# JunzheJosephZhu/DenseMatcher

Hardware: AMD Instinct MI355X
Metric: mesh-pairs/sec at N=2048 D=768 k=128 (higher is better)
Workload: dtype f16; 1 GPU; configs[1]: batch=64 pairs, N=2048, D=768, k=128 functional-map solve; pairs_per_gpu=64, N=2048, D=768, k=128, basis_dtype=float64, parallelism=pairs sharded over 1 GPU(s), one process per GPU, no data-path collective, process_group_size=1

## Files before the change

densematcher_amd/csrc/dm_ctx.hip:

```cpp
#include <stdarg.h>

#include "dm_internal.h"

int dm_fail(dm_ctx* ctx, int code, const char* fmt, ...) {
    char buf[1024];
    va_list ap;
    va_start(ap, fmt);
    vsnprintf(buf, sizeof(buf), fmt, ap);
    va_end(ap);
    if (ctx) ctx->err = buf;
    return code;
}

static thread_local std::string g_create_err = "null context";

static int create_fail(const char* what, hipError_t e) {
    char buf[512];
    snprintf(buf, sizeof(buf), "dm_create: %s%s%s", what, e != hipSuccess ? ": " : "", e != hipSuccess ? hipGetErrorString(e) : "");
    g_create_err = buf;
    return DM_EHIP;
}

extern "C" int dm_create(int device, void* hip_stream, dm_ctx** out) {
    if (!out) return DM_EINVAL;
// ... 11 lines not shown
        char buf[300];
        snprintf(buf, sizeof(buf), "device is %s, libdensematch is built for gfx950 only", prop.gcnArchName);
        return create_fail(buf, hipSuccess);
    }
    dm_ctx* ctx = new dm_ctx();
    ctx->n_cu = prop.multiProcessorCount;
    ctx->device = device;
    ctx->stream = (hipStream_t)hip_stream;
    *out = ctx;
    return DM_OK;
}

extern "C" int dm_destroy(dm_ctx* ctx) {
    if (!ctx) return DM_EINVAL;
    (void)hipSetDevice(ctx->device);
    (void)hipStreamSynchronize(ctx->stream);
    for (hipEvent_t e : ctx->prof_events) (void)hipEventDestroy(e);
    if (ctx->ws) (void)hipFree(ctx->ws);
    if (ctx->gram_keep) (void)hipFree(ctx->gram_keep);
    for (auto& e : ctx->stats) { if (e.buf[0]) (void)hipFree(e.buf[0]); }
    if (ctx->pinned_words) (void)hipHostFree(ctx->pinned_words);
    if (ctx->pinned_event) (void)hipEventDestroy(ctx->pinned_event);
    delete ctx;
    return DM_OK;
}

int dm_pinned_words(dm_ctx* ctx, int32_t** words, hipEvent_t* ev) {
    if (!ctx->pinned_words) DM_CHECK_HIP(ctx, hipHostMalloc((void**)&ctx->pinned_words, 64 * sizeof(int32_t), hipHostMallocDefault));
    if (!ctx->pinned_event) DM_CHECK_HIP(ctx, hipEventCreateWithFlags(&ctx->pinned_event, hipEventDisableTiming));
    *words = ctx->pinned_words; *ev = ctx->pinned_event;
    return DM_OK;
}

#ifdef DM_EXPERIMENTS
#include <stdlib.h>
int dm_knob(const char* env_name, int dflt) {
    const char* e = getenv(env_name);
    return e ? atoi(e) : dflt;
}
#endif

extern "C" int dm_set_option(dm_ctx* ctx, const char* name, int value) {
    if (!ctx || !name) return DM_EINVAL;
    const std::string n = name;
    if (n == "simnn_pipe") ctx->opt_simnn_pipe = value;
    else if (n == "knn_split") ctx->opt_knn_split = value;
    else if (n == "solve_packed") ctx->opt_solve_packed = value;
    else if (n == "solve_reg") ctx->opt_solve_reg = value;
    else if (n == "simnn_band") ctx->opt_simnn_band = value;
    else if (n == "simnn_big") ctx->opt_simnn_big = value;
    else if (n == "simnn_prio") ctx->opt_simnn_prio = value;
    else if (n == "fit_mfma") ctx->opt_fit_mfma = value;
    else if (n == "solve_pcg") ctx->opt_solve_pcg = value;
    else if (n == "basis_stats") { ctx->opt_basis_stats = value; for (auto& e : ctx->stats) e.valid = false; }
    else if (n == "lsa_reg") ctx->opt_lsa_reg = value;
    else if (n == "p2p_split") ctx->opt_p2p_split = value;
    else if (n == "simnn_persist") ctx->opt_simnn_persist = value;
    else if (n == "p2pfm_direct") ctx->opt_p2pfm_direct = value;
    else if (n == "zoomout_fused") ctx->opt_zoomout_fused = value;
    else if (n == "simnn1_wt") ctx->opt_simnn1_wt = value;
    else if (n == "zoomout_sub_fused") ctx->opt_zoomout_sub_fused = value;
    else if (n == "fps_heat_route") ctx->opt_fps_heat_route = value;
    else if (n == "graph_geod_device") ctx->opt_graph_geod_device = value;
    else if (n == "fmn_eig_route") ctx->opt_fmn_eig_route = value;
    else if (n == "proj_onepass") ctx->opt_proj_onepass = value;
    else if (n == "energy_keep_gram") { ctx->opt_energy_keep_gram = value; ctx->gram_valid = false; }
    else return dm_fail(ctx, DM_EINVAL, "dm_set_option: unknown option '%s'", name);
    return DM_OK;
}

extern "C" const char* dm_last_error(const dm_ctx* ctx) { return ctx ? ctx->err.c_str() : g_create_err.c_str(); }
extern "C" const char* dm_version(void) { return DM_VERSION_STRING; }
extern "C" size_t dm_workspace_bytes(const dm_ctx* ctx) { return ctx ? ctx->ws_bytes : 0; }

dm_ctx::basis_stat* dm_stat_entry(dm_ctx* ctx, const void* ptr, int B, int N, int k, int ld, int esz, int n) {
    for (auto& e : ctx->stats)
        if (e.ptr == ptr && e.B == B && e.N == N && e.k == k && e.ld == ld && e.esz == esz && e.n == n && e.buf[0]) return &e;
    dm_ctx::basis_stat& e = ctx->stats[ctx->stats_next];
    ctx->stats_next = (ctx->stats_next + 1) % 4;
    const size_t need = (size_t)B * n * 8;
    if (!e.buf[0] || (size_t)e.B * e.n * 8 < need) {
        if (e.buf[0]) { (void)hipStreamSynchronize(ctx->stream); (void)hipFree(e.buf[0]); e.buf[0] = e.buf[1] = nullptr; }
        void* p = nullptr;
        if (hipMalloc(&p, 2 * dm_align_up(need)) != hipSuccess) { e.ptr = nullptr; return nullptr; }
        e.buf[0] = (double*)p;
        e.buf[1] = (double*)((char*)p + dm_align_up(need));
    } else {
        e.buf[1] = (double*)((char*)e.buf[0] + dm_align_up(need));
    }
    e.ptr = ptr; e.B = B; e.N = N; e.k = k; e.ld = ld; e.esz = esz; e.n = n; e.cur = 0; e.valid = false;
    return &e;
}

int dm_ws_reserve(dm_ctx* ctx, size_t total_bytes) {
    ctx->ws_off = 0;
    ctx->last_flag_counts = nullptr;
    ctx->last_flag_sets = 0;
    total_bytes = dm_align_up(total_bytes + 4096, 1 << 20);
    if (total_bytes <= ctx->ws_bytes) return DM_OK;
    DM_CHECK_HIP(ctx, hipSetDevice(ctx->device));
    if (ctx->ws) {
        DM_CHECK_HIP(ctx, hipStreamSynchronize(ctx->stream));
        DM_CHECK_HIP(ctx, hipFree(ctx->ws));
        ctx->ws = nullptr;
        ctx->ws_bytes = 0;
    }
// ... 106 lines not shown
```

densematcher_amd/csrc/dm_fmap.hip:

```cpp
#include <stdlib.h>

#include "dm_gemm_f64.h"
#include "dm_internal.h"
#include "dm_pcg.h"

struct OutProj {
    float* direct;
    double* partial;
    int B, k, D;
    __device__ __forceinline__ void store(int b, int split, int m, int c, double v) const {
        if (direct) direct[((long long)b * k + m) * D + c] = (float)v;
        else partial[(((long long)split * B + b) * k + m) * D + c] = v;
    }
};

__global__ __launch_bounds__(256) void splitk_reduce_f32_kernel(const double* __restrict__ partial, int nsplit,
                                                                long long n, float* __restrict__ out) {
    const long long i = (long long)blockIdx.x * 256 + threadIdx.x;
    if (i >= n) return;
    double s = 0.0;
    for (int q = 0; q < nsplit; ++q) s += partial[(long long)q * n + i];
    out[i] = (float)s;
}

// ... 587 lines not shown
                    const double* Tik = T + sl(I, K);
#pragma unroll
                    for (int ii = 0; ii < 16; ++ii) a0 = fma(Tik[k * 16 + ii], xv[I * 16 + ii], a0);
                }
                rhs[K * 16 + k] -= a0;
            }
            __syncthreads();
            for (int q = t; q < r1n * 128; q += 256) reinterpret_cast<f64x2*>(T)[q] = reinterpret_cast<const f64x2*>(my_spill)[q];
            __syncthreads();
            blocked_back_subst(T, TriSlots{}, rhs, xv, NA, t);
            if (t == 0) Crow[0] = ci0;
            for (int c = t; c < n; c += 256) Crow[c + 1] = xv[c];
        } else {
            if (t == 0) atomicMax(&info[b], i + 1);
            for (int c = t; c < k1; c += 256) Crow[c] = (c == 0) ? ci0 : 0.0;
        }
        __syncthreads();
    }
}

#include "dm_chol_reg.h"
#ifndef DM_SOLVE_REG_EV
#define DM_SOLVE_REG_EV 3
#endif

constexpr int solve_reg_ev(int NBT) { return NBT == 8 ? DM_SOLVE_REG_EV : 0; }
constexpr size_t solve_reg_lds(int NBT) {
    const size_t img = (size_t)(NBT * (NBT + 1) / 2) * 256 * sizeof(double);
    const size_t ev = (size_t)4 * dmreg::ev_slot(NBT, solve_reg_ev(NBT), solve_reg_ev(NBT) + 1) * 256 * sizeof(double);
    return img > ev ? img : ev;
}

template <int NBT>
__global__ __launch_bounds__(256, 1) void fmap_solve_reg_kernel(const double* __restrict__ PQ, const double* __restrict__ Timg,
                                                                const double* __restrict__ lam1, const double* __restrict__ lam2,
                                                                const double* __restrict__ c00, double w_lap, int k1, int k2, int NBimg,
                                                                long long nsys, double* __restrict__ C, int32_t* __restrict__ info,
                                                                const int32_t* __restrict__ only_if, int only_ng) {
    const int lane = threadIdx.x & 63, wave = threadIdx.x >> 6;
    const long long sys0 = (long long)blockIdx.x * 4;
    if (only_if && !pcg_flagged(only_if, only_ng, (int)(sys0 / k2)) && !pcg_flagged(only_if, only_ng, (int)(min(sys0 + 3, nsys - 1) / k2))) return;
    const long long sys = min(sys0 + wave, nsys - 1);
    const int b = (int)(sys / k2), i = (int)(sys - (long long)b * k2);
    const int n = k1 - 1, c = lane & 15, g = lane >> 4;
    const double* P = PQ + (long long)b * (k1 + k2) * k1;
    const double* Q = P + (long long)k1 * k1;
    const double* l1 = lam1 + (long long)b * k1;
    const double* l2 = lam2 + (long long)b * k2;
    extern __shared__ __attribute__((aligned(16))) double sh_dyn[];
    f64x4 T[NBT * (NBT + 1) / 2];
    {
        const int nblk = NBimg * (NBimg + 1) / 2;
        const bool one_pair = (int)(sys0 / k2) == (int)(min(sys0 + 3, nsys - 1) / k2);
        const double* imgb = Timg + (long long)b * nblk * 256;
        if (one_pair) {
            const f64x2* src = reinterpret_cast<const f64x2*>(imgb);
            f64x2* dst = reinterpret_cast<f64x2*>(sh_dyn);
            for (int q = threadIdx.x; q < nblk * 128; q += 256) dst[q] = src[q];
            __syncthreads();
        }
#pragma unroll
        for (int I = 0; I < NBT; ++I)
#pragma unroll
            for (int K = 0; K <= I; ++K) {
                f64x4 v = {0.0, 0.0, 0.0, 0.0};
                if (I < NBimg) {
                    if (one_pair) {
#pragma unroll
                        for (int r = 0; r < 4; ++r) v[r] = sh_dyn[dmreg::blk(I, K) * 256 + 64 * r + lane];
                    } else {
#pragma unroll
                        for (int r = 0; r < 4; ++r) v[r] = imgb[(long long)dmreg::blk(I, K) * 256 + 64 * r + lane];
                    }
                }
                T[dmreg::blk(I, K)] = v;
            }
        __syncthreads();
    }
    double mx = -DM_INF_F64;
    for (int q = lane; q < k1; q += 64) mx = fmax(mx, l1[q]);
    for (int q = lane; q < k2; q += 64) mx = fmax(mx, l2[q]);
#pragma unroll
    for (int off = 32; off > 0; off >>= 1) mx = fmax(mx, __shfl_xor(mx, off));
    const double scale = mx;
    const double ci0 = (i == 0) ? c00[b] : 0.0;
    const double l2i = l2[i] / scale;
#pragma unroll
    for (int I = 0; I < NBT; ++I) {
        const int idx = I * 16 + c;
        double pen = 1.0;
        if (idx < n) {
            const double d = l1[idx + 1] / scale - l2i;
            pen = w_lap * (d * d);
        }
        const bool mine = g == (c & 3);
#pragma unroll
        for (int r = 0; r < 4; ++r) {
            const bool hit = mine && (c >> 2) == r;
            const double cur = T[dmreg::blk(I, I)][r];
            T[dmreg::blk(I, I)][r] = hit ? (idx < n ? cur + pen : 1.0) : cur;
        }
    }
    double* Crow = C + ((long long)b * k2 + i) * k1;
    __shared__ double sh_rhs[4][NBT * 16];
    for (int q = lane; q < NBT * 16; q += 64)
        sh_rhs[wave][q] = (q < n) ? Q[(long long)i * k1 + (q + 1)] - (i == 0 ? P[(long long)(q + 1) * k1] * ci0 : 0.0) : 0.0;
    auto rhs = [&](int J) {
        f64x4 rv = {0.0, 0.0, 0.0, 0.0};
        if (c == 0) {
#pragma unroll
            for (int r = 0; r < 4; ++r) rv[r] = sh_rhs[wave][J * 16 + g + 4 * r];
        }
        return rv;
    };
    auto store = [&](int J, const f64x4& x) {
        if (c == 0) {
#pragma unroll
            for (int r = 0; r < 4; ++r) {
                const int ix = J * 16 + g + 4 * r;
                if (ix < n) Crow[ix + 1] = x[r];
            }
        }
    };
    constexpr int EV = solve_reg_ev(NBT);
    if (sys0 + wave >= nsys) return;
    const bool solved = dmreg::solve<NBT, EV>(T, rhs, store, lane, sh_dyn + wave * (dmreg::ev_slot(NBT, EV, EV + 1) * 256));
    if (!solved) {
        if (lane == 0) atomicMax(&info[b], i + 1);
        for (int q = lane; q < k1; q += 64) Crow[q] = (q == 0) ? ci0 : 0.0;
        return;
    }
    if (lane == 0) Crow[0] = ci0;
}

static size_t fmap_solve_ws(const dm_ctx* ctx, int B, int k1, int k2) {
    const size_t pq_bytes = (size_t)B * (k1 + k2) * k1 * 8;
    const int n = k1 - 1, NB = (n + 15) / 16;
    const bool two_phase = (NB == 12 || NB == 13) && !ctx->opt_solve_packed;
    const bool blocked = ((n >= 1 && NB <= 11) && !ctx->opt_solve_packed) || two_phase;
    const size_t img_bytes = blocked ? (size_t)B * (NB * (NB + 1) / 2) * 256 * 8 : 0;
    const int NA = (NB + 1) / 2, grid2 = ctx->n_cu > 0 ? ctx->n_cu : 256;
    const size_t spill_bytes = two_phase ? (size_t)grid2 * (NA * (NA + 1) / 2) * 256 * 8 : 0;
    const size_t pcgs_bytes = (ctx->opt_solve_pcg && n > 128 && n <= 256) ? pcgs_image_bytes(B, n) : 0;
    return dm_align_up(pq_bytes) + dm_align_up(img_bytes) + dm_align_up(spill_bytes) + dm_align_up((size_t)B * dm_cdiv(k2, 32) * 4) + dm_align_up(pcgs_bytes) + 4096;
}

static inline bool fmap_solve_pcg_ok(const dm_ctx* ctx, int k1, int k2) {
    const int n = k1 - 1;
    return ctx->opt_solve_pcg && ctx->opt_solve_reg && !ctx->opt_solve_packed && n >= 65 && n <= 128 && k2 % 4 == 0;
}

template <class OPA, class OPB>
static int fmap_solve_core(dm_ctx* ctx, int B, int k1, int k2, int D, const OPA& opa, const OPB& opb,
                           const double* lam1, const double* lam2, const double* c00, double w_descr, double w_lap,
                           double* C, int32_t* info) {
    const size_t pq_bytes = (size_t)B * (k1 + k2) * k1 * 8;
    const int n = k1 - 1;
    const int NB = (n + 15) / 16;
    const bool two_phase = (NB == 12 || NB == 13) && !ctx->opt_solve_packed;
    const bool blocked = ((n >= 1 && NB <= 11) && !ctx->opt_solve_packed) || two_phase;
    const size_t img_bytes = blocked ? (size_t)B * (NB * (NB + 1) / 2) * 256 * 8 : 0;
    const int NA = (NB + 1) / 2;
    const int grid2 = ctx->n_cu > 0 ? ctx->n_cu : 256;
    const size_t spill_bytes = two_phase ? (size_t)grid2 * (NA * (NA + 1) / 2) * 256 * 8 : 0;
    int rc = DM_OK;
    double* PQ = (double*)dm_ws_take(ctx, pq_bytes);
    double* Timg = blocked ? (double*)dm_ws_take(ctx, img_bytes) : nullptr;
    double* spill = two_phase ? (double*)dm_ws_take(ctx, spill_bytes) : nullptr;
    if (!PQ || (blocked && !Timg) || (two_phase && !spill)) return dm_fail(ctx, DM_ENOMEM, "fmap_solve: workspace not reserved");
    if (blocked) DM_CHECK_HIP(ctx, hipMemsetAsync(Timg, 0, img_bytes, ctx->stream));
    const bool pcg_small = blocked && !two_phase && NB <= 8 && ctx->opt_solve_reg && fmap_solve_pcg_ok(ctx, k1, k2);
    const bool pcg_big = (two_phase || (blocked && NB >= 9)) && ctx->opt_solve_pcg && !ctx->opt_solve_packed;
    if (!pcg_small && !pcg_big) DM_CHECK_HIP(ctx, hipMemsetAsync(info, 0, (size_t)B * sizeof(int32_t), ctx->stream));

    OutScaled out{PQ, (long long)(k1 + k2) * k1, k1, w_descr, Timg, (long long)(NB * (NB + 1) / 2) * 256, k1};
    dim3 grid(dm_cdiv(k1 + k2, NT_T) * dm_cdiv(k1, NT_T), 1, B);
    switch (dm_knob("DM_GRAM_NPRE", 2)) {
        case 1: DM_LAUNCH(ctx, "gram_nt_f64", (gemm_nt_f64<OPA, OPB, OutScaled, 1>), grid, dim3(256), 0, opa, opb, out, k1 + k2, k1, D); break;
        case 4: DM_LAUNCH(ctx, "gram_nt_f64", (gemm_nt_f64<OPA, OPB, OutScaled, 4>), grid, dim3(256), 0, opa, opb, out, k1 + k2, k1, D); break;
        case 3: DM_LAUNCH(ctx, "gram_nt_f64", (gemm_nt_f64<OPA, OPB, OutScaled, 3>), grid, dim3(256), 0, opa, opb, out, k1 + k2, k1, D); break;
        default: DM_LAUNCH(ctx, "gram_nt_f64", (gemm_nt_f64<OPA, OPB, OutScaled, 2, true>), dim3(grid.x * (unsigned)B), dim3(256), 0, opa, opb, out, k1 + k2, k1, D); break;
    }

    const int32_t* only_if_big = nullptr;
    const int only_ng = dm_cdiv(k2, PCG_NS);
    if (pcg_big) {
        int32_t* fb = (int32_t*)dm_ws_take(ctx, (size_t)B * only_ng * 4);
        double* img = (double*)dm_ws_take(ctx, pcgs_image_bytes(B, n));
        if (!fb || !img) return dm_fail(ctx, DM_ENOMEM, "fmap_solve: workspace not reserved");
        const int NTp = (n + 15) / 16, KSP = pcgs_ksp(n), ngroups = dm_cdiv(k2, PCG_NS);
        DM_LAUNCH(ctx, "fmap_solve_pcg_pack", pcgs_pack_kernel, dim3(64, B), dim3(256), 0, (const double*)PQ, k1, k2, NTp, KSP, img);
        const size_t lds_pcg = pcg_lds_bytes(PCGS_NT, PCGS_NW);
        rc = dm_grant_lds(ctx, (const void*)fmap_solve_pcgs_kernel, lds_pcg);
        if (rc) return rc;
        DM_LAUNCH(ctx, "fmap_solve_pcg", fmap_solve_pcgs_kernel, dim3((unsigned)(B * ngroups)), dim3(64 * PCGS_NW), lds_pcg, (const double*)PQ,
                  (const double*)img, lam1, lam2, c00, w_lap, k1, k2, ngroups, NTp, KSP, 1e-22, 48, 6, 3e-4, C, fb, info);
        only_if_big = fb;
    }
    if (two_phase) {
        const int NBr = NB - NA;
        const size_t lds = ((size_t)(NA * (NA + 1) / 2 + NBr * NA + 2) * 256 + 2 * NB * 16 + 8) * sizeof(double) + (96 + 16 + 128) * sizeof(int);
        rc = dm_grant_lds(ctx, (const void*)fmap_solve_2phase_kernel, lds);
        if (rc) return rc;
        const long long nsys = (long long)B * k2;
        DM_LAUNCH(ctx, "fmap_solve_chol", fmap_solve_2phase_kernel, dim3((unsigned)(nsys < grid2 ? nsys : grid2)), dim3(256), lds, PQ, Timg,
                  lam1, lam2, c00, w_lap, k1, k2, NB, B, spill, C, info, only_if_big, only_ng);
        return DM_OK;
    }
    if (blocked && !two_phase && NB <= 8 && ctx->opt_solve_reg) {
        const long long nsys = (long long)B * k2;
        const dim3 grid((unsigned)((nsys + 3) / 4));
        const int32_t* only_if = nullptr;
        if (pcg_small) {
            int32_t* fb = (int32_t*)dm_ws_take(ctx, (size_t)B * only_ng * 4);
            if (!fb) return dm_fail(ctx, DM_ENOMEM, "fmap_solve: workspace not reserved");
            const int ngroups = dm_cdiv(k2, PCG_NS);
            const size_t lds_pcg = pcg_lds_bytes(8, 4);
            rc = dm_grant_lds(ctx, (const void*)fmap_solve_pcg_kernel<8, 4>, lds_pcg);
            if (rc) return rc;
            DM_LAUNCH(ctx, "fmap_solve_pcg", (fmap_solve_pcg_kernel<8, 4>), dim3((unsigned)(B * ngroups)), dim3(256), lds_pcg, PQ, lam1, lam2, c00,
                      w_lap, k1, k2, ngroups, 1e-22, 48, 6, 3e-4, C, fb, info);
            only_if = fb;
        }
#define DM_SOLVE_REG(NBT_)                                                                                             \
        {                                                                                                              \
            rc = dm_grant_lds(ctx, (const void*)fmap_solve_reg_kernel<NBT_>, solve_reg_lds(NBT_));                     \
            if (rc) return rc;                                                                                         \
            DM_LAUNCH(ctx, "fmap_solve_chol", fmap_solve_reg_kernel<NBT_>, grid, dim3(256), solve_reg_lds(NBT_), PQ, Timg, lam1, lam2, \
                      c00, w_lap, k1, k2, NB, nsys, C, info, only_if, only_ng);                                        \
        }
        if (NB <= 2) DM_SOLVE_REG(2)
        else if (NB <= 4) DM_SOLVE_REG(4)
        else if (NB <= 6) DM_SOLVE_REG(6)
        else DM_SOLVE_REG(8)
#undef DM_SOLVE_REG
        return DM_OK;
    }
    if (blocked) {
        const size_t lds = ((size_t)(NB * (NB + 1) / 2 + 2) * 256 + 2 * NB * 16 + 16 + 8) * sizeof(double);
        rc = dm_grant_lds(ctx, (const void*)fmap_solve_blocked_kernel, lds);
        if (rc) return rc;
        DM_LAUNCH(ctx, "fmap_solve_chol", fmap_solve_blocked_kernel, dim3(k2, B), dim3(256), lds, PQ, Timg, lam1, lam2, c00,
                  w_lap, k1, k2, NB, C, info, only_if_big, only_ng);
        return DM_OK;
    }
    const size_t lds = ((size_t)(n + 1) * (n + 2) / 2 + (n + 1 < 16 ? 16 : n + 1) + 4) * sizeof(double);
    rc = dm_grant_lds(ctx, (const void*)fmap_solve_kernel, lds);
    if (rc) return rc;
    DM_LAUNCH(ctx, "fmap_solve_chol", fmap_solve_kernel, dim3(k2, B), dim3(SP_NT), lds, PQ, lam1, lam2, c00, w_lap, k1, k2,
              C, info, dm_knob("DM_SOLVE_DEBUG", 0));
    return DM_OK;
}

extern "C" int dm_fmap_solve(dm_ctx* ctx, int B, int k1, int k2, int D, const float* A, const float* Bm,
                             const double* lam1, const double* lam2, const double* c00, double w_descr, double w_lap,
                             double* C, int32_t* info) {
    if (!ctx) return DM_EINVAL;
    DM_REQUIRE(ctx, B > 0 && k1 > 0 && k2 > 0 && D > 0, "sizes must be positive");
    DM_REQUIRE(ctx, A && Bm && lam1 && lam2 && c00 && C && info, "null pointer");
    DM_REQUIRE(ctx, k1 <= 200, "k1 > 200 does not fit the in-LDS solver");
    DM_REQUIRE(ctx, w_descr >= 0.0 && w_lap >= 0.0 && (w_descr > 0.0 || w_lap > 0.0), "weights must be >= 0 and not both 0");
    DM_CHECK_HIP(ctx, hipSetDevice(ctx->device));
    int rc = dm_ws_reserve(ctx, fmap_solve_ws(ctx, B, k1, k2));
    if (rc) return rc;
    KRowsStackedF32 opa{A, Bm, k1, k2, D};
    KRowsF32 opb{A, (long long)k1 * D, D, k1, D};
    return fmap_solve_core(ctx, B, k1, k2, D, opa, opb, lam1, lam2, c00, w_descr, w_lap, C, info);
}

template <typename TR>
static int fmap_fit_impl(dm_ctx* ctx, int B, int N1, int N2, int D, int k1, int k2, const TR* Phi1, int ld1, const TR* Phi2, int ld2,
                         const TR* mass1, const TR* mass2, const void* F1, const void* F2, const double* lam1, const double* lam2,
                         double w_descr, double w_lap, double* C, int32_t* info) {
    if (!ctx) return DM_EINVAL;
// ... 44 lines not shown
```

densematcher_amd/csrc/dm_internal.h:

```cpp
#pragma once

#include <hip/hip_runtime.h>
#include <stdint.h>
#include <stdio.h>
#include <string.h>

#include <string>
#include <unordered_map>
#include <vector>

#include "densematch.h"

#define DM_VERSION_STRING "densematch 0.5.0 (gfx950, abi 6)"

struct dm_ctx {
    int device = 0;
    hipStream_t stream = nullptr;
    std::string err;

    char* ws = nullptr;
    size_t ws_bytes = 0;
    size_t ws_off = 0;

    std::string prof_name;
    std::vector<hipEvent_t> prof_events;
    std::vector<const char*> prof_names;
    std::vector<const char*> prof_syms;
    size_t prof_used = 0;

    std::unordered_map<const void*, size_t> lds_granted;

    int opt_simnn_pipe = 1;
    int opt_knn_split = 1;
    int opt_solve_packed = 0;
    int opt_proj_onepass = 1;
    int opt_fit_mfma = 1;
    int opt_simnn_prio = 0;
    int opt_simnn_big = 0;
    int opt_simnn_band = 4;
    int opt_lsa_reg = 2;
    int opt_solve_pcg = 1;
    int opt_solve_reg = 1;
    int opt_p2p_split = 2;
    int opt_simnn_persist = 1;
    int opt_p2pfm_direct = 1;
    int opt_simnn1_wt = 4;
    int opt_zoomout_fused = 1;
    int opt_zoomout_sub_fused = 1;
    int opt_fps_heat_route = 0;
    int opt_graph_geod_device = 1;
    int opt_fmn_eig_route = 0;
    int opt_energy_keep_gram = 0;
    double* gram_keep = nullptr;
    size_t gram_keep_bytes = 0;
    const void* gram_key_ptr[5] = {nullptr, nullptr, nullptr, nullptr, nullptr};
    int gram_key_dim[6] = {0, 0, 0, 0, 0, 0};
    bool gram_valid = false;
    bool gram_sums_valid = false;
    int n_cu = 0;
    int32_t* pinned_words = nullptr;
    hipEvent_t pinned_event = nullptr;
    struct basis_stat { const void* ptr = nullptr; int B = 0, N = 0, k = 0, ld = 0, esz = 0, n = 0; double* buf[2] = {nullptr, nullptr}; int cur = 0; bool valid = false; };
    basis_stat stats[4];
    int stats_next = 0;
    int opt_basis_stats = 1;
    const int32_t* last_flag_counts = nullptr;
    int last_flag_sets = 0;
};

#ifdef DM_EXPERIMENTS
int dm_knob(const char* env_name, int dflt);
#else
static inline int dm_knob(const char*, int dflt) { return dflt; }
#endif

int dm_fail(dm_ctx* ctx, int code, const char* fmt, ...);
int dm_pinned_words(dm_ctx* ctx, int32_t** words, hipEvent_t* ev);
int dm_grant_lds(dm_ctx* ctx, const void* func, size_t bytes);

#define DM_CHECK_HIP(ctx, expr)                                                        \
    do {                                                                               \
        hipError_t _e = (expr);                                                        \
        if (_e != hipSuccess)                                                          \
            return dm_fail(ctx, DM_EHIP, "%s failed: %s (%s:%d)", #expr,               \
                           hipGetErrorString(_e), __FILE__, __LINE__);                 \
    } while (0)

#define DM_REQUIRE(ctx, cond, msg)                                                     \
    do {                                                                               \
        if (!(cond)) return dm_fail(ctx, DM_EINVAL, "%s: requirement failed: %s (%s)", \
                                    __func__, #cond, msg);                             \
    } while (0)

int dm_ws_reserve(dm_ctx* ctx, size_t total_bytes);
// ... 187 lines not shown
```

densematcher_amd/csrc/dm_p2p.hip:

```cpp
#include <stdlib.h>

#include "dm_gemm_f64.h"
#include "dm_internal.h"
#include "dm_split.h"
#include "dm_indicator_dev.h"

static inline int pad_to(int x, int m) { return (x + m - 1) / m * m; }

template <typename Tin>
__global__ __launch_bounds__(256) void phiT_kernel(const Tin* __restrict__ Phi, int N, int k, int ld,
                                                   double* __restrict__ out, int kpad, int Npad, double* __restrict__ amax) {
    __shared__ Tin tile[64][65];
    const int b = blockIdx.z;
    const int i0 = blockIdx.x * 64, c0 = blockIdx.y * 64;
    const Tin* P = Phi + (long long)b * N * ld;
    double* O = out + (long long)b * kpad * Npad;
    const int tx = threadIdx.x & 63, ty = threadIdx.x >> 6;
    double m = 0.0;
    for (int r = ty; r < 64; r += 4) {
        const int i = i0 + r, c = c0 + tx;
        const Tin v = (i < N && c < k) ? P[(long long)i * ld + c] : (Tin)0;
        tile[r][tx] = v;
        m = fmax(m, fabs((double)v));
    }
// ... 673 lines not shown
                  p.tilesM, a.N1, a.N1pad, 1, a.ind12);
    }
    return DM_OK;
}

template <typename TR>
static int fm_to_p2p_impl(dm_ctx* ctx, int B, int N1, int N2, int k1, int k2, const TR* Phi1, int ld1,
                          const TR* Phi2, int ld2, const TR* mass1_in, const double* C, int32_t* knn21,
                          int32_t* knn12, int32_t* ind21, int32_t* ind12) {
    if (!ctx) return DM_EINVAL;
    DM_REQUIRE(ctx, B > 0 && N1 > 0 && N2 > 0 && k1 > 0 && k2 > 0, "sizes must be positive");
    DM_REQUIRE(ctx, Phi1 && Phi2 && C, "null input");
    DM_REQUIRE(ctx, ld1 >= k1 && ld2 >= k2, "eigenvector row stride smaller than the map size");
    DM_REQUIRE(ctx, (!ind21 && !ind12) || mass1_in, "mass1 is needed for the indicator maps");
    if (!knn21 && !knn12 && !ind21 && !ind12) return DM_OK;
    DM_CHECK_HIP(ctx, hipSetDevice(ctx->device));

    const int N1pad = pad_to(N1, GT), N2pad = pad_to(N2, GT);
    const int Kpad = pad_to(k2, GBK);
    const int K1pad = pad_to(k1, GBK);
    const bool all = knn12 || ind21 || ind12;
    const size_t bytes_E2 = 0;
    const bool split = knn21 && knn12 && ind21 && ind12 && mass1_in && dm_fm_split_ok(ctx, N2, N1, k2);
    const size_t bytes_AT = split ? 0 : (size_t)B * Kpad * N2pad * 8, bytes_BT = (size_t)B * Kpad * N1pad * 8;
    const int nS = dm_cdiv(N1pad, DM_EMB_COLS), nT = dm_cdiv(N2pad, DM_EMB_COLS);
    const size_t bytes_amax = (size_t)B * (nS + nT) * 8;
    const size_t bytes_zero = split ? dm_fm_split_zero_bytes(B) : 0;
    const size_t need = dm_align_up(bytes_AT) + dm_align_up(bytes_BT) + dm_align_up(bytes_E2) +
                        dm_align_up((size_t)B * N1pad * 8) + dm_align_up((size_t)B * N2pad * 8) +
                        dm_align_up((size_t)B * N1 * 8) + dm_align_up(bytes_amax) + dm_align_up(bytes_zero) +
                        (split ? dm_fm_split_ws_bytes(B, N2, N1, k2) : dm_gred_ws_bytes(B, N2, N1));
    int rc = dm_ws_reserve(ctx, need);
    if (rc) return rc;
    double* AT = bytes_AT ? (double*)dm_ws_take(ctx, bytes_AT) : nullptr;
    double* BT = (double*)dm_ws_take(ctx, bytes_BT);
    double* E2 = bytes_E2 ? (double*)dm_ws_take(ctx, bytes_E2) : nullptr;
    double* n1 = (double*)dm_ws_take(ctx, (size_t)B * N1pad * 8);
    double* n2 = (double*)dm_ws_take(ctx, (size_t)B * N2pad * 8);
    double* amaxS = (double*)dm_ws_take(ctx, bytes_amax);
    void* zeroed = bytes_zero ? dm_ws_take(ctx, bytes_zero) : nullptr;
    double* massbuf = (double*)dm_ws_take(ctx, (size_t)B * N1 * 8);
    const double* mass1 = nullptr;
    rc = dm_widen_mass(ctx, (long long)B * N1, mass1_in, massbuf, &mass1);
    if (rc) return rc;
    double* amaxT = amaxS + (size_t)B * nS;
    if ((bytes_AT && !AT) || !BT || (bytes_E2 && !E2) || !n1 || !n2 || !amaxS || (bytes_zero && !zeroed))
        return dm_fail(ctx, DM_ENOMEM, "fm_to_p2p: workspace not reserved");
    if (zeroed) DM_CHECK_HIP(ctx, hipMemsetAsync(zeroed, 0, bytes_zero, ctx->stream));

    if (!split) {
        rc = dm_launch_phiT(ctx, B, N2, k2, Phi2, ld2, AT, Kpad, N2pad, (double*)nullptr);
        if (rc) return rc;
    }
    rc = dm_launch_embed(ctx, B, N1, k2, k1, Phi1, ld1, C, k1, (long long)k2 * k1, 0, BT, Kpad, N1pad, n1, 1, amaxS);
    if (rc) return rc;
    dm_ctx::basis_stat* st = (split && ctx->opt_basis_stats) ? dm_stat_entry(ctx, Phi2, B, N2, k2, ld2, (int)sizeof(TR), 1) : nullptr;
    dm_fm_split_pre pre{nullptr, false, nullptr, nullptr};
    dm_embed_fx fx{nullptr, 0, 0, nullptr, 0, nullptr};
    if (split) {
        int D_ = 0, R2_ = 0;
        pre.Fx = dm_fm_split_take_fx(ctx, B, N2, k2, &D_, &R2_);
        if (!pre.Fx) return dm_fail(ctx, DM_ENOMEM, "fm_to_p2p: workspace not reserved");
        if (st) {
            if (st->valid) { fx.F = pre.Fx; fx.D = D_; fx.rows_out = R2_; fx.hint = st->buf[st->cur]; fx.n_hint = 1; pre.built = true; pre.hint = fx.hint; }
            pre.pair_out = st->buf[st->cur ^ 1];
        }
    }
    if (all) {
        rc = dm_launch_embed(ctx, B, N2, k1, k2, Phi2, ld2, C, k1, (long long)k2 * k1, 1, (double*)nullptr, K1pad, N2pad, n2, 1,
                             (double*)nullptr, split ? amaxT : nullptr, (split && st) ? &fx : nullptr);
        if (rc) return rc;
        if (st) { st->cur ^= 1; st->valid = true; }
    }
    dm_gred_args a;
    a.B = B; a.N2 = N2; a.N1 = N1; a.Kloop = Kpad;
    a.AT = AT; a.N2pad = N2pad; a.BT = BT; a.N1pad = N1pad; a.Kpad = Kpad;
    a.n1 = n1; a.n2 = all ? n2 : nullptr; a.mass1 = mass1;
    if (all && !mass1) {
        if (!massbuf) return dm_fail(ctx, DM_ENOMEM, "fm_to_p2p: workspace not reserved");
        DM_CHECK_HIP(ctx, hipMemsetAsync(massbuf, 0, (size_t)B * N1 * 8, ctx->stream));
        a.mass1 = massbuf;
    }
    a.knn21 = knn21; a.knn12 = knn12; a.ind21 = ind21; a.ind12 = ind12;
    ctx->last_flag_counts = nullptr;
    if (split) { a.Ktrue = k2; return dm_launch_fm_split<TR>(ctx, a, amaxS, nS, amaxT, nT, zeroed, Phi2, ld2, &pre); }
    return dm_launch_gred(ctx, a);
}
extern "C" int dm_fm_to_p2p(dm_ctx* ctx, int B, int N1, int N2, int k1, int k2, const float* Phi1, int ld1,
                            const float* Phi2, int ld2, const float* mass1, const double* C, int32_t* knn21,
                            int32_t* knn12, int32_t* ind21, int32_t* ind12) {
    return fm_to_p2p_impl<float>(ctx, B, N1, N2, k1, k2, Phi1, ld1, Phi2, ld2, mass1, C, knn21, knn12, ind21, ind12);
}
extern "C" int dm_fm_to_p2p_f64(dm_ctx* ctx, int B, int N1, int N2, int k1, int k2, const double* Phi1, int ld1,
                                const double* Phi2, int ld2, const double* mass1, const double* C, int32_t* knn21,
                                int32_t* knn12, int32_t* ind21, int32_t* ind12) {
    return fm_to_p2p_impl<double>(ctx, B, N1, N2, k1, k2, Phi1, ld1, Phi2, ld2, mass1, C, knn21, knn12, ind21, ind12);
}

extern "C" int dm_fm_to_p2p_uses_split(const dm_ctx* ctx, int N2, int N1, int k) {
    return (ctx && dm_fm_split_ok(ctx, N2, N1, k)) ? ctx->opt_p2p_split : 0;
}

extern "C" int dm_knn_query_f64(dm_ctx* ctx, int B, int nx, int ny, int p, const double* X, const double* Y, int32_t* out) {
    if (!ctx) return DM_EINVAL;
    DM_REQUIRE(ctx, B > 0 && nx > 0 && ny > 0 && p > 0, "sizes must be positive");
    DM_REQUIRE(ctx, X && Y && out, "null pointer");
    DM_CHECK_HIP(ctx, hipSetDevice(ctx->device));
    const int nxpad = pad_to(nx, GT), nypad = pad_to(ny, GT), Kpad = pad_to(p, GBK);
    const size_t bA = (size_t)B * Kpad * nypad * 8, bB = (size_t)B * Kpad * nxpad * 8;
    int rc = dm_ws_reserve(ctx, dm_align_up(bA) + dm_align_up(bB) + dm_align_up((size_t)B * nxpad * 8) + dm_gred_ws_bytes(B, ny, nx) +
                                dm_knn_split_prep_bytes(B, ny, p) + dm_knn_split_ws_bytes(B, ny, nx, p) +
                                dm_align_up((size_t)B * (nxpad / 256 + 1) * 8));
    if (rc) return rc;
    double* AT = (double*)dm_ws_take(ctx, bA);
    double* BT = (double*)dm_ws_take(ctx, bB);
    double* n1 = (double*)dm_ws_take(ctx, (size_t)B * nxpad * 8);
    double* amaxS = (double*)dm_ws_take(ctx, (size_t)B * (nxpad / 256 + 1) * 8);
    rc = launch_transpose_f64(ctx, B, ny, p, Y, p, AT, Kpad, nypad);
    if (rc) return rc;
    rc = launch_transpose_f64(ctx, B, nx, p, X, p, BT, Kpad, nxpad);
    if (rc) return rc;
    DM_LAUNCH(ctx, "colnorm", colnorm_kernel, dim3(dm_cdiv(nxpad, 256), B), dim3(256), 0, BT, p, Kpad, nxpad, n1, amaxS);
    dm_knn_split_state knn;
    rc = dm_knn_split_prepare(ctx, B, ny, nypad, Kpad, p, AT, &knn);
    if (rc) return rc;
    dm_gred_args a;
// ... 73 lines not shown
```

densematcher_amd/csrc/dm_pcg.h:

```cpp
#pragma once
#include "dm_device.h"

constexpr int PCG_NS = 32;

__device__ __forceinline__ bool pcg_flagged(const int32_t* __restrict__ flags, int ng, int b) {
    int f = 0;
    for (int q = 0; q < ng; ++q) f |= flags[(long long)b * ng + q];
    return f != 0;
}
constexpr int PCG_LDP = 48;

static inline size_t pcg_lds_bytes(int NT, int NW) { return ((size_t)NT * 16 * PCG_LDP + 2 * NW * PCG_NS + 64) * sizeof(double); }

__device__ __forceinline__ double pcg_rows4_sum(double v) {
    unsigned lo = (unsigned)__double2loint(v), hi = (unsigned)__double2hiint(v);
    const auto a = __builtin_amdgcn_permlane16_swap(lo, lo, false, false);
    const auto b = __builtin_amdgcn_permlane16_swap(hi, hi, false, false);
    const double e = __hiloint2double((int)b[0], (int)a[0]) + __hiloint2double((int)b[1], (int)a[1]);
    lo = (unsigned)__double2loint(e); hi = (unsigned)__double2hiint(e);
    const auto c = __builtin_amdgcn_permlane32_swap(lo, lo, false, false);
    const auto d = __builtin_amdgcn_permlane32_swap(hi, hi, false, false);
    return __hiloint2double((int)d[0], (int)c[0]) + __hiloint2double((int)d[1], (int)c[1]);
}

template <int NW>
__device__ __forceinline__ void pcg_colsum(double (&v)[2], double* red, int wave, int lane) {
#pragma unroll
    for (int ct = 0; ct < 2; ++ct) v[ct] = pcg_rows4_sum(v[ct]);
    if (lane < 16) { red[wave * PCG_NS + lane] = v[0]; red[wave * PCG_NS + 16 + lane] = v[1]; }
    __syncthreads();
    const int l15 = lane & 15;
#pragma unroll
    for (int ct = 0; ct < 2; ++ct) {
        double s = red[ct * 16 + l15];
#pragma unroll
        for (int w = 1; w < NW; ++w) s += red[w * PCG_NS + ct * 16 + l15];
        v[ct] = s;
    }
}

template <int NT, int NW>
__global__ __launch_bounds__(64 * NW, 1) void fmap_solve_pcg_kernel(const double* __restrict__ PQ, const double* __restrict__ lam1,
                                                                    const double* __restrict__ lam2, const double* __restrict__ c00,
                                                                    double w_lap, int k1, int k2, int ngroups, double tol2, int maxit,
                                                                    int slow_it, double slow_tol2,
                                                                    double* __restrict__ C, int32_t* __restrict__ fallback, int32_t* __restrict__ info) {
    static_assert(NT % NW == 0, "whole tiles per wave");
    constexpr int RTW = NT / NW, KS = NT * 4;
    extern __shared__ __attribute__((aligned(16))) double pcg_sm[];
    double* pL = pcg_sm;
    double* red = pL + NT * 16 * PCG_LDP;
    int* s_notpd = reinterpret_cast<int*>(red + 2 * NW * PCG_NS);
    const int b = (int)blockIdx.x / ngroups, g = (int)blockIdx.x - b * ngroups;
    const int t = threadIdx.x, lane = t & 63, l15 = lane & 15, lg = lane >> 4;
    const int wave = __builtin_amdgcn_readfirstlane(t >> 6);
    const int n = k1 - 1;
    const double* P = PQ + (long long)b * (k1 + k2) * k1;
    const double* Q = P + (long long)k1 * k1;
    const double* l1 = lam1 + (long long)b * k1;
    const double* l2 = lam2 + (long long)b * k2;

    double mx = -DM_INF_F64;
    for (int q = t; q < k1; q += 64 * NW) mx = fmax(mx, l1[q]);
    for (int q = t; q < k2; q += 64 * NW) mx = fmax(mx, l2[q]);
#pragma unroll
    for (int off = 32; off > 0; off >>= 1) mx = fmax(mx, __shfl_xor(mx, off));
    if (lane == 0) red[wave] = mx;
    if (t == 0) *s_notpd = 0;
    __syncthreads();
    double scale = red[0];
#pragma unroll
    for (int w = 1; w < NW; ++w) scale = fmax(scale, red[w]);
    __syncthreads();

    double Pf[RTW][KS];
#pragma unroll
    for (int rt = 0; rt < RTW; ++rt) {
        const int row = 16 * (wave * RTW + rt) + l15;
#pragma unroll
        for (int s = 0; s < KS; ++s) {
            const int col = 4 * s + lg;
            Pf[rt][s] = (row < n && col < n) ? P[(long long)(row + 1) * k1 + col + 1] : 0.0;
        }
    }
    double x[RTW][2][4], r[RTW][2][4], pv[RTW][2][4], minv[RTW][2][4], dd[RTW][2][4];
    double part[2] = {0.0, 0.0};
    bool notpd = false;
#pragma unroll
    for (int ct = 0; ct < 2; ++ct) {
        const int i = g * PCG_NS + ct * 16 + l15;
        const bool iok = i < k2;
        const double l2i = iok ? l2[i] / scale : 0.0;
        const double ci0 = (i == 0) ? c00[b] : 0.0;
#pragma unroll
        for (int rt = 0; rt < RTW; ++rt)
#pragma unroll
            for (int q = 0; q < 4; ++q) {
                const int c = 16 * (wave * RTW + rt) + lg + 4 * q;
                const bool ok = iok && c < n;
                const int cc = ok ? c : 0, ii = ok ? i : 0;
                const double d = l1[cc + 1] / scale - l2i;
                const double dv = w_lap * (d * d);
                const double m = P[(long long)(cc + 1) * (k1 + 1)] + dv;
                const double bv = Q[(long long)ii * k1 + cc + 1] - P[(long long)(cc + 1) * k1] * ci0;
                if (ok && !(m > 0.0)) notpd = true;
                dd[rt][ct][q] = ok ? dv : 0.0;
                minv[rt][ct][q] = (ok && m > 0.0) ? 1.0 / m : 0.0;
                x[rt][ct][q] = 0.0;
                r[rt][ct][q] = ok ? bv : 0.0;
                pv[rt][ct][q] = r[rt][ct][q] * minv[rt][ct][q];
                part[ct] = fma(r[rt][ct][q], pv[rt][ct][q], part[ct]);
            }
    }
    if (notpd) *s_notpd = 1;
    pcg_colsum<NW>(part, red, wave, lane);
    notpd = *s_notpd != 0;
    double rz[2] = {part[0], part[1]}, rz0[2] = {part[0], part[1]};
    int rbuf = 1;
    bool done = false;
    int it = 0;
    for (; it < maxit && !done && !notpd; ++it) {
#pragma unroll
        for (int rt = 0; rt < RTW; ++rt)
#pragma unroll
            for (int ct = 0; ct < 2; ++ct)
#pragma unroll
                for (int q = 0; q < 4; ++q) pL[(16 * (wave * RTW + rt) + lg + 4 * q) * PCG_LDP + ct * 16 + l15] = pv[rt][ct][q];
        __syncthreads();
        f64x4 acc[RTW][2];
#pragma unroll
        for (int rt = 0; rt < RTW; ++rt)
#pragma unroll
            for (int ct = 0; ct < 2; ++ct) acc[rt][ct] = f64x4{0.0, 0.0, 0.0, 0.0};
        constexpr int G = 4, NG = KS / G;
        static_assert(KS % G == 0, "whole groups of k-steps");
        double bq[2][G][2];
#pragma unroll
        for (int u = 0; u < G; ++u) { bq[0][u][0] = pL[(4 * u + lg) * PCG_LDP + l15]; bq[0][u][1] = pL[(4 * u + lg) * PCG_LDP + 16 + l15]; }
#pragma unroll
        for (int gq = 0; gq < NG; ++gq) {
            if (gq + 1 < NG) {
#pragma unroll
                for (int u = 0; u < G; ++u) {
                    const int sn = (gq + 1) * G + u;
                    bq[(gq + 1) & 1][u][0] = pL[(4 * sn + lg) * PCG_LDP + l15];
                    bq[(gq + 1) & 1][u][1] = pL[(4 * sn + lg) * PCG_LDP + 16 + l15];
                }
            }
            __builtin_amdgcn_sched_barrier(0);
#pragma unroll
            for (int u = 0; u < G; ++u) {
                const int s = gq * G + u;
#pragma unroll
                for (int rt = 0; rt < RTW; ++rt) {
                    acc[rt][0] = mfma_f64_16x16x4(Pf[rt][s], bq[gq & 1][u][0], acc[rt][0]);
                    acc[rt][1] = mfma_f64_16x16x4(Pf[rt][s], bq[gq & 1][u][1], acc[rt][1]);
                }
            }
            __builtin_amdgcn_sched_barrier(0);
        }
        part[0] = part[1] = 0.0;
#pragma unroll
        for (int rt = 0; rt < RTW; ++rt)
#pragma unroll
            for (int ct = 0; ct < 2; ++ct)
#pragma unroll
                for (int q = 0; q < 4; ++q) {
                    acc[rt][ct][q] = fma(dd[rt][ct][q], pv[rt][ct][q], acc[rt][ct][q]);
                    part[ct] = fma(pv[rt][ct][q], acc[rt][ct][q], part[ct]);
                }
        pcg_colsum<NW>(part, red + rbuf * NW * PCG_NS, wave, lane);
        rbuf ^= 1;
        double alpha[2];
// ... 273 lines not shown
```

densematcher_amd/engine.py:

```python
import ctypes as C
import types

import numpy as np
import torch

from . import _lib
from ._engine_aggre import _AggreOps
from ._engine_dnet import _DiffusionNetOps
from ._engine_eval import _EvalOps
from ._engine_geodesic import GraphTooWide, _GeodesicOps, heat_geodesic_check
from ._engine_jbu import _JbuOps
from ._engine_lift import _LiftOps
from ._engine_mesh import _MeshOps
from ._engine_network import _NetworkOps
from ._operands import fits_abi, host_ptr, ptr as _ptr


class _KeepAlive(tuple):
    """an argument tuple that also holds the tensors its raw pointers refer to"""


class MatchEngine(_MeshOps, _GeodesicOps, _DiffusionNetOps, _LiftOps, _JbuOps, _AggreOps, _EvalOps, _NetworkOps):
    def __init__(self, device=None, lib_path=None):
        if not torch.cuda.is_available():
# ... 28 lines not shown
            raise RuntimeError("MatchEngine is bound to the stream it was created on; create one engine per stream "
                               "(default_engine() does) instead of calling it under torch.cuda.stream(other)")

    def _dev(self, t, dtype, name):
        self._check_stream()
        if not isinstance(t, torch.Tensor):
            t = torch.as_tensor(t)
        if t.device != self.device or t.dtype != dtype or not t.is_contiguous():
            t = t.to(device=self.device, dtype=dtype).contiguous()
        return t

    def _strided(self, t, dtype, name):
        if not isinstance(t, torch.Tensor) or t.device != self.device or t.dtype != dtype:
            t = self._dev(t, dtype, name)
        else:
            self._check_stream()
        if t.dim() not in (2, 3):
            raise ValueError(f"{name}: expected a (B, N, W) or (N, W) tensor, got {tuple(t.shape)}")
        ld = fits_abi(t)
        return (t, ld) if ld is not None else (t.contiguous(), int(t.shape[-1]))

    def _descr(self, F):
        F = F if isinstance(F, torch.Tensor) else torch.as_tensor(F)
        half = F.dtype == torch.float16
        return self._dev(F, torch.float16 if half else torch.float32, "F"), _lib.DM_F16 if half else _lib.DM_F32

    @staticmethod
    def _raise_not_pd(info):
        bad = torch.nonzero(info).flatten()
        if bad.numel():
            raise _lib.DenseMatchError(
                f"functional-map system not positive definite for pairs {bad.tolist()[:8]} "
                f"(row {int(info[bad[0]]) - 1}): descriptors are rank deficient in the basis and w_lap cannot fix it")

    @staticmethod
    def _raise_lsa(info):
        worst = int(info.max())
        if worst == 2:
            raise ValueError("matrix contains invalid numeric entries")
        if worst == 1:
            raise ValueError("cost matrix is infeasible")

    def _reals(self, *arrays):
        def dt(a):
            return a.dtype if isinstance(a, torch.Tensor) else getattr(a, "dtype", None)
        f64 = any(a is not None and str(dt(a)).endswith("float64") for a in arrays)
        tdt = torch.float64 if f64 else torch.float32
        return ("_f64" if f64 else "",) + tuple(None if a is None else self._dev(a, tdt, "real") for a in arrays)

    def synchronize(self):
        self.stream.synchronize()

    OPTION_DEFAULTS = {"simnn_pipe": 1, "simnn_persist": 1, "knn_split": 1, "p2p_split": 2, "solve_packed": 0, "solve_reg": 1, "simnn_band": 4, "lsa_reg": 2, "simnn_big": 0, "energy_keep_gram": 0,
                       "p2pfm_direct": 1, "zoomout_fused": 1, "proj_onepass": 1, "fit_mfma": 1, "basis_stats": 1, "solve_pcg": 1,
                       "zoomout_sub_fused": 1, "fps_heat_route": 0, "graph_geod_device": 1, "fmn_eig_route": 0}

    def set_option(self, name, value):
        self._chk(self.lib.dm_set_option(self.ctx, name.encode(), int(value)))
        self._options[name] = int(value)

    def get_option(self, name):
        return self._options[name]

    def reset_options(self):
        for k, v in self.OPTION_DEFAULTS.items():
            self.set_option(k, v)

    @staticmethod
    def split_depth(k):
        return max(96, -(-(8 + 3 * k) // 32) * 32)

    def p2p_split_active(self, N2, N1, k):
        return int(self.lib.dm_fm_to_p2p_uses_split(self.ctx, int(N2), int(N1), int(k)))

    def last_requeued_rows(self):
        out = (C.c_int * 4)()
        self._chk(self.lib.dm_last_requeued_rows(self.ctx, out))
        return [int(x) for x in out]

    def workspace_bytes(self):
        return int(self.lib.dm_workspace_bytes(self.ctx))

    def profile_kernel(self, name):
        self._chk(self.lib.dm_profile_kernel(self.ctx, name.encode() if name else None))

    def profile_read(self):
        n, ms = C.c_int(0), C.c_double(0.0)
        self._chk(self.lib.dm_profile_read(self.ctx, C.byref(n), C.byref(ms)))
        return n.value, ms.value

    PEAK_PROBES = {"mfma_f16_zero_operands": 0, "mfma_f16_random_operands": 1, "mfma_f64": 2, "hbm_copy": 3}

    def measure_peak(self, which):
        v = C.c_double(0.0)
        self._chk(self.lib.dm_measure_peak(self.ctx, self.PEAK_PROBES[which], C.byref(v)))
        return v.value

    def profile_report(self, kernels=False):
        buf = C.create_string_buffer(1 << 16)
        self._chk(self.lib.dm_profile_report(self.ctx, buf, len(buf)))
        out = {}
        for line in buf.value.decode().splitlines():
            name, n, ms, syms = line.split("\t")
            out[name] = (int(n), float(ms), tuple(syms.split(";"))) if kernels else (int(n), float(ms))
        return out

    def simnn(self, Ftgt, Fsrc, return_scores=False):
# ... 557 lines not shown
```

Baseline: 62790 mesh-pairs/s.

## Add pipelined PCG variant, build solve image in-kernel, reorder embed launch

```diff
diff --git a/densematcher_amd/csrc/dm_ctx.hip b/densematcher_amd/csrc/dm_ctx.hip
--- a/densematcher_amd/csrc/dm_ctx.hip
+++ b/densematcher_amd/csrc/dm_ctx.hip
@@ -87,6 +87,7 @@
     else if (n == "simnn_prio") ctx->opt_simnn_prio = value;
     else if (n == "fit_mfma") ctx->opt_fit_mfma = value;
     else if (n == "solve_pcg") ctx->opt_solve_pcg = value;
+    else if (n == "pcg_pipeline") ctx->opt_pcg_pipeline = value;
     else if (n == "basis_stats") { ctx->opt_basis_stats = value; for (auto& e : ctx->stats) e.valid = false; }
     else if (n == "lsa_reg") ctx->opt_lsa_reg = value;
     else if (n == "p2p_split") ctx->opt_p2p_split = value;
diff --git a/densematcher_amd/csrc/dm_fmap.hip b/densematcher_amd/csrc/dm_fmap.hip
--- a/densematcher_amd/csrc/dm_fmap.hip
+++ b/densematcher_amd/csrc/dm_fmap.hip
@@ -663,8 +663,22 @@
     {
         const int nblk = NBimg * (NBimg + 1) / 2;
         const bool one_pair = (int)(sys0 / k2) == (int)(min(sys0 + 3, nsys - 1) / k2);
-        const double* imgb = Timg + (long long)b * nblk * 256;
-        if (one_pair) {
+        const double* imgb = Timg ? Timg + (long long)b * nblk * 256 : nullptr;
+        if (!Timg) {
+            const int r15 = threadIdx.x >> 4, c15 = threadIdx.x & 15;
+            double stg[NBT * (NBT + 1) / 2];
+#pragma unroll
+            for (int I = 0; I < NBT; ++I)
+#pragma unroll
+                for (int K = 0; K <= I; ++K) {
+                    const int r = 16 * I + r15, cc = 16 * K + c15;
+                    stg[dmreg::blk(I, K)] = (I < NBimg && r < n && cc < n) ? P[(long long)(r + 1) * k1 + cc + 1] : 0.0;
+                }
+#pragma unroll
+            for (int q = 0; q < NBT * (NBT + 1) / 2; ++q)
+                if (q < nblk) sh_dyn[q * 256 + c15 * 16 + r15] = stg[q];
+            __syncthreads();
+        } else if (one_pair) {
             const f64x2* src = reinterpret_cast<const f64x2*>(imgb);
             f64x2* dst = reinterpret_cast<f64x2*>(sh_dyn);
             for (int q = threadIdx.x; q < nblk * 128; q += 256) dst[q] = src[q];
@@ -676,7 +690,7 @@
             for (int K = 0; K <= I; ++K) {
                 f64x4 v = {0.0, 0.0, 0.0, 0.0};
                 if (I < NBimg) {
-                    if (one_pair) {
+                    if (one_pair || !Timg) {
 #pragma unroll
                         for (int r = 0; r < 4; ++r) v[r] = sh_dyn[dmreg::blk(I, K) * 256 + 64 * r + lane];
                     } else {
@@ -779,9 +793,10 @@
     double* Timg = blocked ? (double*)dm_ws_take(ctx, img_bytes) : nullptr;
     double* spill = two_phase ? (double*)dm_ws_take(ctx, spill_bytes) : nullptr;
     if (!PQ || (blocked && !Timg) || (two_phase && !spill)) return dm_fail(ctx, DM_ENOMEM, "fmap_solve: workspace not reserved");
-    if (blocked) DM_CHECK_HIP(ctx, hipMemsetAsync(Timg, 0, img_bytes, ctx->stream));
     const bool pcg_small = blocked && !two_phase && NB <= 8 && ctx->opt_solve_reg && fmap_solve_pcg_ok(ctx, k1, k2);
     const bool pcg_big = (two_phase || (blocked && NB >= 9)) && ctx->opt_solve_pcg && !ctx->opt_solve_packed;
+    if (pcg_small) Timg = nullptr;
+    if (Timg) DM_CHECK_HIP(ctx, hipMemsetAsync(Timg, 0, img_bytes, ctx->stream));
     if (!pcg_small && !pcg_big) DM_CHECK_HIP(ctx, hipMemsetAsync(info, 0, (size_t)B * sizeof(int32_t), ctx->stream));
 
     OutScaled out{PQ, (long long)(k1 + k2) * k1, k1, w_descr, Timg, (long long)(NB * (NB + 1) / 2) * 256, k1};
@@ -827,10 +842,16 @@
             if (!fb) return dm_fail(ctx, DM_ENOMEM, "fmap_solve: workspace not reserved");
             const int ngroups = dm_cdiv(k2, PCG_NS);
             const size_t lds_pcg = pcg_lds_bytes(8, 4);
-            rc = dm_grant_lds(ctx, (const void*)fmap_solve_pcg_kernel<8, 4>, lds_pcg);
+            rc = ctx->opt_pcg_pipeline ? dm_grant_lds(ctx, (const void*)fmap_solve_pcg_kernel<8, 4, true>, lds_pcg)
+                                       : dm_grant_lds(ctx, (const void*)fmap_solve_pcg_kernel<8, 4>, lds_pcg);
             if (rc) return rc;
-            DM_LAUNCH(ctx, "fmap_solve_pcg", (fmap_solve_pcg_kernel<8, 4>), dim3((unsigned)(B * ngroups)), dim3(256), lds_pcg, PQ, lam1, lam2, c00,
-                      w_lap, k1, k2, ngroups, 1e-22, 48, 6, 3e-4, C, fb, info);
+            if (!ctx->opt_pcg_pipeline) {
+                DM_LAUNCH(ctx, "fmap_solve_pcg", (fmap_solve_pcg_kernel<8, 4>), dim3((unsigned)(B * ngroups)), dim3(256), lds_pcg, PQ, lam1, lam2, c00,
+                          w_lap, k1, k2, ngroups, 1e-22, 48, 6, 3e-4, C, fb, info);
+            } else {
+                DM_LAUNCH(ctx, "fmap_solve_pcg", (fmap_solve_pcg_kernel<8, 4, true>), dim3((unsigned)(B * ngroups)), dim3(256), lds_pcg, PQ, lam1, lam2, c00,
+                          w_lap, k1, k2, ngroups, 1e-22, 48, 6, 3e-4, C, fb, info);
+            }
             only_if = fb;
         }
 #define DM_SOLVE_REG(NBT_)                                                                                             \
diff --git a/densematcher_amd/csrc/dm_internal.h b/densematcher_amd/csrc/dm_internal.h
--- a/densematcher_amd/csrc/dm_internal.h
+++ b/densematcher_amd/csrc/dm_internal.h
@@ -40,6 +40,7 @@
     int opt_simnn_band = 4;
     int opt_lsa_reg = 2;
     int opt_solve_pcg = 1;
+    int opt_pcg_pipeline = 0;
     int opt_solve_reg = 1;
     int opt_p2p_split = 2;
     int opt_simnn_persist = 1;
diff --git a/densematcher_amd/csrc/dm_p2p.hip b/densematcher_amd/csrc/dm_p2p.hip
--- a/densematcher_amd/csrc/dm_p2p.hip
+++ b/densematcher_amd/csrc/dm_p2p.hip
@@ -749,8 +749,6 @@
         rc = dm_launch_phiT(ctx, B, N2, k2, Phi2, ld2, AT, Kpad, N2pad, (double*)nullptr);
         if (rc) return rc;
     }
-    rc = dm_launch_embed(ctx, B, N1, k2, k1, Phi1, ld1, C, k1, (long long)k2 * k1, 0, BT, Kpad, N1pad, n1, 1, amaxS);
-    if (rc) return rc;
     dm_ctx::basis_stat* st = (split && ctx->opt_basis_stats) ? dm_stat_entry(ctx, Phi2, B, N2, k2, ld2, (int)sizeof(TR), 1) : nullptr;
     dm_fm_split_pre pre{nullptr, false, nullptr, nullptr};
     dm_embed_fx fx{nullptr, 0, 0, nullptr, 0, nullptr};
@@ -769,6 +767,8 @@
         if (rc) return rc;
         if (st) { st->cur ^= 1; st->valid = true; }
     }
+    rc = dm_launch_embed(ctx, B, N1, k2, k1, Phi1, ld1, C, k1, (long long)k2 * k1, 0, BT, Kpad, N1pad, n1, 1, amaxS);
+    if (rc) return rc;
     dm_gred_args a;
     a.B = B; a.N2 = N2; a.N1 = N1; a.Kloop = Kpad;
     a.AT = AT; a.N2pad = N2pad; a.BT = BT; a.N1pad = N1pad; a.Kpad = Kpad;
diff --git a/densematcher_amd/csrc/dm_pcg.h b/densematcher_amd/csrc/dm_pcg.h
--- a/densematcher_amd/csrc/dm_pcg.h
+++ b/densematcher_amd/csrc/dm_pcg.h
@@ -39,7 +39,15 @@
     }
 }
 
-template <int NT, int NW>
+template <int NW>
+__device__ __forceinline__ void pcg_colsum_put(double v, double* red, int wave, int lane) {
+    v = pcg_rows4_sum(v);
+    if (lane < 16) red[wave * 16 + lane] = v;
+}
+
+template <int V> struct pcg_ic { static constexpr int v = V; };
+
+template <int NT, int NW, bool PIPE = false>
 __global__ __launch_bounds__(64 * NW, 1) void fmap_solve_pcg_kernel(const double* __restrict__ PQ, const double* __restrict__ lam1,
                                                                     const double* __restrict__ lam2, const double* __restrict__ c00,
                                                                     double w_lap, int k1, int k2, int ngroups, double tol2, int maxit,
@@ -119,6 +127,152 @@
     int rbuf = 1;
     bool done = false;
     int it = 0;
+    if constexpr (PIPE) {
+        constexpr int G = 4, NG = KS / G;
+        static_assert(KS % G == 0 && NG == 8, "eight slices per product");
+        double bq[2][G];
+        f64x4 acc[RTW][2];
+        bool conv[2] = {false, false};
+        double s = 0.0, alpha = 0.0, beta = 0.0, rp[NW];
+        auto put_p = [&](auto YC) __attribute__((always_inline)) {
+            constexpr int Y = decltype(YC)::v;
+#pragma unroll
+            for (int rt = 0; rt < RTW; ++rt)
+#pragma unroll
+                for (int q = 0; q < 4; ++q) pL[(16 * (wave * RTW + rt) + lg + 4 * q) * PCG_LDP + Y * 16 + l15] = pv[rt][Y][q];
+        };
+        auto bload = [&](auto XC, auto GC) __attribute__((always_inline)) {
+            constexpr int X = decltype(XC)::v, GQ = decltype(GC)::v;
+#pragma unroll
+            for (int u = 0; u < G; ++u) bq[GQ & 1][u] = pL[(4 * (GQ * G + u) + lg) * PCG_LDP + X * 16 + l15];
+        };
+        auto mgrp = [&](auto XC, auto GC) __attribute__((always_inline)) {
+            constexpr int X = decltype(XC)::v, GQ = decltype(GC)::v;
+#pragma unroll
+            for (int u = 0; u < G; ++u)
+#pragma unroll
+                for (int rt = 0; rt < RTW; ++rt) acc[rt][X] = mfma_f64_16x16x4(Pf[rt][GQ * G + u], bq[GQ & 1][u], acc[rt][X]);
+        };
+        auto red_get = [&](const double* rb) __attribute__((always_inline)) {
+#pragma unroll
+            for (int w = 0; w < NW; ++w) rp[w] = rb[w * 16 + l15];
+        };
+        auto red_sum = [&]() __attribute__((always_inline)) {
+            s = rp[0];
+#pragma unroll
+            for (int w = 1; w < NW; ++w) s += rp[w];
+        };
+        auto v1 = [&](auto YC) __attribute__((always_inline)) {
+            constexpr int Y = decltype(YC)::v;
+            s = 0.0;
+#pragma unroll
+            for (int rt = 0; rt < RTW; ++rt)
+#pragma unroll
+                for (int q = 0; q < 4; ++q) {
+                    acc[rt][Y][q] = fma(dd[rt][Y][q], pv[rt][Y][q], acc[rt][Y][q]);
+                    s = fma(pv[rt][Y][q], acc[rt][Y][q], s);
+                }
+            pcg_colsum_put<NW>(s, red + 2 * Y * NW * 16, wave, lane);
+        };
+        auto v2a = [&](auto YC) __attribute__((always_inline)) {
+            constexpr int Y = decltype(YC)::v;
+            red_sum();
+            if (rz[Y] > 0.0 && !(s > 0.0)) notpd = true;
+            alpha = (s > 0.0) ? rz[Y] / s : 0.0;
+        };
+        auto v2b = [&](auto YC) __attribute__((always_inline)) {
+            constexpr int Y = decltype(YC)::v;
+            s = 0.0;
+#pragma unroll
+            for (int rt = 0; rt < RTW; ++rt)
+#pragma unroll
+                for (int q = 0; q < 4; ++q) {
+                    x[rt][Y][q] = fma(alpha, pv[rt][Y][q], x[rt][Y][q]);
+                    r[rt][Y][q] = fma(-alpha, acc[rt][Y][q], r[rt][Y][q]);
+                    const double z = r[rt][Y][q] * minv[rt][Y][q];
+                    s = fma(r[rt][Y][q], z, s);
+                    acc[rt][Y][q] = z;
+                }
+            pcg_colsum_put<NW>(s, red + (2 * Y + 1) * NW * 16, wave, lane);
+        };
+        auto v3a = [&](auto YC) __attribute__((always_inline)) {
+            constexpr int Y = decltype(YC)::v;
+            red_sum();
+            beta = rz[Y] > 0.0 ? s / rz[Y] : 0.0;
+            rz[Y] = s;
+            conv[Y] = !(rz[Y] > tol2 * rz0[Y]);
+        };
+        auto v3b = [&](auto YC) __attribute__((always_inline)) {
+            constexpr int Y = decltype(YC)::v;
+#pragma unroll
+            for (int rt = 0; rt < RTW; ++rt)
+#pragma unroll
+                for (int q = 0; q < 4; ++q) pv[rt][Y][q] = fma(beta, pv[rt][Y][q], acc[rt][Y][q]);
+            put_p(YC);
+        };
+#define PCG_SB __builtin_amdgcn_sched_barrier(0)
+        auto half = [&](auto XC, auto VC) __attribute__((always_inline)) {
+            constexpr int X = decltype(XC)::v, Y = 1 - X;
+            constexpr bool VEC = decltype(VC)::v != 0;
+            const pcg_ic<Y> YC;
+            const double* redY = red + 2 * Y * NW * 16;
+#pragma unroll
+            for (int rt = 0; rt < RTW; ++rt) acc[rt][X] = f64x4{0.0, 0.0, 0.0, 0.0};
+            bload(XC, pcg_ic<1>{});
+            if constexpr (VEC) red_get(redY);
+            PCG_SB; mgrp(XC, pcg_ic<0>{}); PCG_SB;
+            bload(XC, pcg_ic<2>{}); PCG_SB;
+            mgrp(XC, pcg_ic<1>{});
+            if constexpr (VEC) v2a(YC);
+            PCG_SB;
+            bload(XC, pcg_ic<3>{}); PCG_SB;
+            mgrp(XC, pcg_ic<2>{});
+            if constexpr (VEC) v2b(YC);
+            PCG_SB;
+            if constexpr (VEC) __syncthreads();
+            bload(XC, pcg_ic<4>{});
+            if constexpr (VEC) red_get(redY + NW * 16);
+            PCG_SB; mgrp(XC, pcg_ic<3>{}); PCG_SB;
+            bload(XC, pcg_ic<5>{}); PCG_SB;
+            mgrp(XC, pcg_ic<4>{});
+            if constexpr (VEC) v3a(YC);
+            PCG_SB;
+            bload(XC, pcg_ic<6>{}); PCG_SB;
+            mgrp(XC, pcg_ic<5>{});
+            if constexpr (VEC) v3b(YC);
+            PCG_SB;
+            bload(XC, pcg_ic<7>{}); PCG_SB;
+            mgrp(XC, pcg_ic<6>{}); PCG_SB;
+            mgrp(XC, pcg_ic<7>{});
+            v1(XC);
+            PCG_SB;
+            __syncthreads();
+            bload(YC, pcg_ic<0>{}); PCG_SB;
+        };
+#undef PCG_SB
+        if (maxit > 0 && !notpd) {
+            put_p(pcg_ic<0>{});
+            put_p(pcg_ic<1>{});
+            __syncthreads();
+            bload(pcg_ic<0>{}, pcg_ic<0>{});
+            half(pcg_ic<0>{}, pcg_ic<0>{});
+            for (;;) {
+                half(pcg_ic<1>{}, pcg_ic<1>{});
+                half(pcg_ic<0>{}, pcg_ic<1>{});
+                done = __all(conv[0] && conv[1]) != 0;
+                notpd = __any(notpd) != 0;
+                if (notpd) break;
+                if (it + 1 == slow_it) {
+                    bool slow = false;
+#pragma unroll
+                    for (int ct = 0; ct < 2; ++ct) slow = slow || (rz[ct] > slow_tol2 * rz0[ct]);
+                    if (__any(slow)) break;
+                }
+                ++it;
+                if (!(it < maxit) || done) break;
+            }
+        }
+    } else
     for (; it < maxit && !done && !notpd; ++it) {
 #pragma unroll
         for (int rt = 0; rt < RTW; ++rt)
diff --git a/densematcher_amd/engine.py b/densematcher_amd/engine.py
--- a/densematcher_amd/engine.py
+++ b/densematcher_amd/engine.py
@@ -104,7 +104,7 @@
         self.stream.synchronize()
 
     OPTION_DEFAULTS = {"simnn_pipe": 1, "simnn_persist": 1, "knn_split": 1, "p2p_split": 2, "solve_packed": 0, "solve_reg": 1, "simnn_band": 4, "lsa_reg": 2, "simnn_big": 0, "energy_keep_gram": 0,
-                       "p2pfm_direct": 1, "zoomout_fused": 1, "proj_onepass": 1, "fit_mfma": 1, "basis_stats": 1, "solve_pcg": 1,
+                       "p2pfm_direct": 1, "zoomout_fused": 1, "proj_onepass": 1, "fit_mfma": 1, "basis_stats": 1, "solve_pcg": 1, "pcg_pipeline": 0,
                        "zoomout_sub_fused": 1, "fps_heat_route": 0, "graph_geod_device": 1, "fmn_eig_route": 0}
 
     def set_option(self, name, value):
```

Result: no change. 62600 mesh-pairs/s (-0.3%).
